# zehuichen123/Graph-DETR4D

Hardware: AMD Instinct MI355X
Metric: decoder_samples_per_sec_900q_T4 (higher is better)
Workload: dtype f32 (bf16x3 GEMMs)

## Files before the change

graph-detr4d_amd/_lib.py:

```python
import ctypes
import os
import threading

_HERE = os.path.dirname(os.path.abspath(__file__))
LIB_PATH = os.environ.get('GD4D_LIB_PATH') or os.path.join(_HERE, 'libgd4d.so')
ABI_VERSION = 56
PIXEL_MAJOR, HEAD_MAJOR = 0, 1

F32, BF16, F16 = 0, 1, 2

_c = ctypes
_vp, _i, _f = _c.c_void_p, _c.c_int, _c.c_float

SIGNATURES = {
    'gd4d_abi_version': (_i, []),
    'gd4d_error_string': (_c.c_char_p, [_i]),
    'gd4d_last_hip_error': (_c.c_char_p, []),
    'gd4d_trace_enable': (_i, [_vp]),
    'gd4d_cross_attn_fwd': (_i, [_vp, _vp, _vp, _vp, _vp, _vp, _vp, _vp, _f, _f, _vp, _vp, _vp,
                                 _i, _i, _i, _i, _i, _i, _i, _i, _i, _i, _vp, _vp]),
    'gd4d_pyramid_channels_last_fwd': (_i, [_vp, _vp, _vp, _i, _i, _i, _i, _i, _i, _vp]),
    'gd4d_cross_attn_agg_fwd': (_i, [_vp] * 8 + [_f, _f] + [_vp] * 4 + [_i] * 9 + [_vp] * 5),
    'gd4d_cross_attn_plan_bytes': (_c.c_size_t, [_i] * 5),
    'gd4d_cross_attn_plan_fwd': (_i, [_vp] * 6 + [_f, _f, _vp, _vp, _c.c_int64, _vp, _c.c_size_t, _vp, _vp, _vp] + [_i] * 7 + [_vp, _vp]),
# ... 40 lines not shown
    'gd4d_linear_fwd': (_i, [_vp] * 7 + [_i] * 9 + [_vp, _vp]),
    'gd4d_linear_group_fwd': (_i, [_vp] * 6 + [_i] * 4 + [_vp, _vp]),
    'gd4d_linear_ln_fwd': (_i, [_vp] * 9 + [_i] * 5 + [_f] + [_i] * 4 + [_vp]),
    'gd4d_small_linear_layernorm_fwd': (_i, [_vp] * 6 + [_i, _i, _i, _f, _i, _vp]),
    'gd4d_layernorm_fwd': (_i, [_vp] * 5 + [_i, _i, _f, _i, _vp]),
    'gd4d_mha_core_fwd': (_i, [_vp] * 5 + [_i] * 10 + [_f, _vp, _f, _vp, _vp]),
    'gd4d_mha_core_bwd': (_i, [_vp] * 11 + [_i] * 14 + [_f, _f, _vp, _vp]),
    'gd4d_mha_core_bwd_fill': (_i, [_vp] * 11 + [_i] * 14 + [_f, _f, _vp] + [_vp, _i, _vp, _vp] + [_i] * 4 + [_vp]),
    'gd4d_layernorm_bwd_workspace_bytes': (_c.c_size_t, [_i, _i]),
    'gd4d_layernorm_bwd': (_i, [_vp] * 9 + [_c.c_size_t, _i, _i, _f, _i, _vp]),
    'gd4d_inverse_sigmoid_fwd': (_i, [_vp, _vp, _c.c_int64, _vp]),
    'gd4d_inverse_sigmoid_bwd': (_i, [_vp, _vp, _vp, _vp, ctypes.c_int64, _vp]),
    'gd4d_layernorm_bwd_reduce_group': (_i, [_vp] * 4 + [_i, _i, _vp]),
    'gd4d_refine_reference_fwd': (_i, [_vp, _vp, _vp, _i, _i, _vp]),
    'gd4d_frustum_pe_input_fwd': (_i, [_vp, _vp, _vp, _i, _i, _i, _i, _f, _f, _f, _vp, _i, _i, _vp]),
    'gd4d_se_fuse_chlast_fwd': (_i, [_vp] * 5 + [_i] * 7 + [_vp]),
    'gd4d_sine_pe3d_fwd': (_i, [_vp, _vp, _vp, _vp, _vp, _i, _i, _i, _i, _i, _vp]),
    'gd4d_se_fuse_fwd': (_i, [_vp, _vp, _vp, _vp, _vp, _c.c_size_t, _vp]),
    'gd4d_split_bf16_fwd': (_i, [_vp, _vp, _vp, _c.c_size_t, _vp]),
    'gd4d_gemm_bf16x3_fwd': (_i, [_vp] * 5 + [_i] * 6 + [_vp]),
    'gd4d_image_job_bytes': (ctypes.c_size_t, []),
    'gd4d_chain_weight_image_group': (_i, [_vp, _i, _i, _vp]),
    'gd4d_gemm_tn_bf16x3_workspace_bytes': (ctypes.c_size_t, [ctypes.c_longlong, _i, _i]),
    'gd4d_gemm_tn_bf16x3': (_i, [_vp] * 5 + [ctypes.c_longlong] + [_i] * 5 + [_vp]),
    'gd4d_se_fuse_chlast_bwd': (_i, [_vp] * 6 + [_i] * 5 + [_vp]),
    'gd4d_knn_farthest_fwd': (_i, [_vp, _vp, _i, _i, _i, _i, _vp]),
    'gd4d_edge_conv_max_fwd': (_i, [_vp] * 6 + [_i] * 5 + [_vp]),
    'gd4d_box_head_fwd': (_i, [_vp, _vp, _vp, _f, _vp, _i, _i, _vp]),
    'gd4d_nms_free_decode_fwd': (_i, [_vp, _vp, _vp, _f, _vp, _vp, _vp, _vp, _i, _i, _i, _i, _i, _vp]),
    'gd4d_value_proj_multi_fwd': (_i, [_vp, _vp, _vp, _vp, _vp, _i, _i, _i, _i, _i, _i, _i, _i, _i, _vp, _c.c_size_t, _i, _vp]),
    'gd4d_chain_op_bytes': (_c.c_size_t, []),
    'gd4d_row_chain_fwd': (_i, [_vp, _i, _i, _vp]),
    'gd4d_row_chain2_fwd': (_i, [_vp, _i, _vp, _i, _i, _vp]),
    'gd4d_mha_core_presplit_fwd': (_i, [_vp] * 4 + [_i] * 5 + [_c.c_longlong, _c.c_longlong, _vp, _i, _f, _vp, _f, _vp, _vp]),
    'gd4d_xcd_placement_probe': (_i, [_vp, _i, _vp]),
    'gd4d_mlp2_image_bytes': (_c.c_size_t, [_i] * 3),
    'gd4d_mlp2_image': (_i, [_vp, _vp, _vp, _i, _i, _i, _vp, _vp]),
    'gd4d_mlp2_bf16x3_fwd': (_i, [_vp] * 4 + [_i] * 6 + [_vp]),
    'gd4d_mlp2_se_fuse_fwd': (_i, [_vp, _vp, _i, _i, _vp, _vp, _vp, _vp, _vp, _i, _i, _vp]),
    'gd4d_mlp2_frustum_fwd': (_i, [_vp, _vp, _i, _i, _c.c_float, _c.c_float, _i, _c.c_float, _vp, _vp, _vp, _vp, _i, _i, _vp]),
    'gd4d_mlp2_pe_se_fwd': (_i, [_vp, _vp, _vp, _i, _i, _c.c_float, _c.c_float, _i, _c.c_float, _vp, _vp, _vp, _i, _vp, _vp, _i, _vp, _vp,
                                  _vp, _vp]),
    'gd4d_adamw_flat_workspace_bytes': (_c.c_size_t, []),
    'gd4d_adamw_flat': (_i, [_vp] * 6 + [_c.c_size_t, _c.c_int64] + [_f] * 6 + [_vp]),
    'gd4d_adamw_recipe_flat_workspace_bytes': (_c.c_size_t, []),
    'gd4d_adamw_recipe_flat_state_bytes': (_c.c_size_t, []),
    'gd4d_adamw_recipe_flat': (_i, [_vp] * 5 + [_c.c_size_t, _vp, _c.c_size_t, _c.c_int64, _vp, _vp, _vp, _i, _vp]),
    'gd4d_chain_weight_image_bytes': (_c.c_size_t, [_i, _i]),
    'gd4d_chain_weight_image': (_i, [_vp, _i, _i, _vp, _vp]),
    'gd4d_chain_weight_image_exact_bytes': (_c.c_size_t, [_i, _i]),
    'gd4d_chain_weight_image_exact': (_i, [_vp, _i, _i, _vp, _vp]),
    'gd4d_linear_sum_assignment_batch': (_i, [_vp] * 4 + [_i, _vp, _vp, _i]),
    'gd4d_hungarian_assign_workspace_bytes': (_c.c_size_t, [_i] * 4),
    'gd4d_hungarian_assign_fwd': (_i, [_vp] * 5 + [_c.c_size_t] + [_i] * 5 + [_vp]),
    'gd4d_hungarian_assign_branches_workspace_bytes': (_c.c_size_t, [_i] * 5),
    'gd4d_hungarian_assign_branches_fwd': (_i, [_vp] * 9 + [_c.c_size_t] + [_i] * 8 + [_vp]),
    'gd4d_match_cost_fwd': (_i, [_vp] * 6 + [_i] * 8 + [_f] * 3 + [_vp]),
    'gd4d_head_loss_fwd_bwd': (_i, [_vp] * 10 + [_i] * 7 + [_f] * 3 + [_vp]),
    'gd4d_linear_bwd_weight': (_i, [_vp] * 4 + [_i] * 6 + [_vp]),
    'gd4d_linear_bwd_weight_group': (_i, [_vp] * 5 + [_i, _i, _vp]),
    'gd4d_value_proj_bwd_input': (_i, [_vp, _vp, _vp, _vp, _i, _i, _i, _i, _vp]),
    'gd4d_value_proj_bwd_weight_workspace_bytes': (_c.c_size_t, []),
    'gd4d_value_proj_bwd_weight': (_i, [_vp] * 6 + [_c.c_size_t, _i, _i, _i, _vp]),
    'gd4d_depth_net_image_bytes': (_c.c_size_t, [_i]),
    'gd4d_depth_net_image': (_i, [_vp, _i, _vp, _vp]),
    'gd4d_cam_gate_fwd': (_i, [_vp, _vp, _i, _i, _f] + [_vp] * 8 + [_i, _vp, _vp]),
# ... 117 lines not shown
```

graph-detr4d_amd/csrc/gd4d_rowchain.hip:

```cpp
#include <stdlib.h>

#include "gd4d_common.h"
#include "gd4d_bf16x3.h"
#include "gd4d_pyramid_fill.h"
#include "gd4d_mha_dropout.h"
#include "gd4d_value_proj_body.h"

namespace gd4d {

GD4D_TRACE_UNIT(rowchain)

constexpr int RC_M = 16;
#ifndef RC_WAVES_N
#define RC_WAVES_N 8
#endif
#ifndef RC_TILES_N
#define RC_TILES_N 2
#endif
constexpr int RC_WAVES = RC_WAVES_N;
#ifndef RC_KPERM
#define RC_KPERM 1
#endif
#ifndef RC_LD_N
#define RC_LD_N 520
// ... 526 lines not shown
  for (int r = 0; r < RC_ROWS_PER_WAVE; ++r) {
    const int m = min(m0 + RC_ROWS_PER_WAVE * wave + r, M - 1);
#pragma unroll
    for (int cb = 0; cb < 2; ++cb) {
      const int n = min(256 * cb + 4 * lane, N - 4);
      va[r][cb] = ga ? *reinterpret_cast<const float4*>(ga + (size_t)m * lda + n) : make_float4(0.f, 0.f, 0.f, 0.f);
      vb[r][cb] = gb ? *reinterpret_cast<const float4*>(gb + (size_t)m * ldb + n) : make_float4(0.f, 0.f, 0.f, 0.f);
    }
  }
#pragma unroll
  for (int r = 0; r < RC_ROWS_PER_WAVE; ++r) {
    const int row = RC_ROWS_PER_WAVE * wave + r;
#pragma unroll
    for (int cb = 0; cb < 2; ++cb) {
      const int n = 256 * cb + 4 * lane;
      if (n >= N) continue;
      float4 v = va[r][cb];
      if (!IS_ADD && (op.flags & GD4D_CHAIN_INV_SIGMOID)) { v.x = inv_sigmoid(v.x); v.y = inv_sigmoid(v.y); v.z = inv_sigmoid(v.z); v.w = inv_sigmoid(v.w); }
      v.x += vb[r][cb].x; v.y += vb[r][cb].y; v.z += vb[r][cb].z; v.w += vb[r][cb].w;
      if (IS_ADD) {
        const float4 s0 = *reinterpret_cast<const float4*>(&bufs[op.src][row][n]);
        v.x += s0.x; v.y += s0.y; v.z += s0.z; v.w += s0.w;
        if (op.res >= 0) {
          const float4 s1 = *reinterpret_cast<const float4*>(&bufs[op.res][row][n]);
          v.x += s1.x; v.y += s1.y; v.z += s1.z; v.w += s1.w;
        }
      }
      *reinterpret_cast<float4*>(&bufs[op.dst][row][(IS_ADD ? 0 : op.dst_col) + n]) = v;
      if (TRAIN && op.gout && m0 + row < M) *reinterpret_cast<float4*>(op.gout + (size_t)(m0 + row) * op.ldg + n) = v;
    }
  }
}

struct ChainProgram {
  int nops, M, nops2, split;
  ChainOp ops[GD4D_CHAIN_MAX_OPS];
};

#if defined(__HIP_DEVICE_COMPILE__)
typedef const __attribute__((address_space(4))) ChainProgram* rc_prog_ptr_t;
#else
typedef const ChainProgram* rc_prog_ptr_t;
#endif

template <bool TRAIN>
__device__ __forceinline__ void row_chain_body(const rc_prog_ptr_t pp, const int bx) {
  const int M = pp->M, split = pp->split;
  const int blocks = (M + RC_M - 1) / RC_M;
  if (split > 0 && bx >= blocks && bx < split) return;
  const bool second = split > 0 && bx >= split;
  const int op_base = second ? pp->nops : 0;
  const int nops = second ? pp->nops2 : pp->nops;
  const int wg = second ? bx - split : bx;
  const int wg_lo = second ? split : 0, wg_hi = wg_lo + blocks;
  extern __shared__ __attribute__((aligned(16))) char rc_smem[];
  float (*bufs)[RC_M][RC_LD] = reinterpret_cast<float (*)[RC_M][RC_LD]>(rc_smem);
  const int tid = threadIdx.x, lane = tid & 63, wave = tid >> 6;
  const int m0 = wg * RC_M;
  trace_mark_if(g_trace_rowchain, (second ? 7ull : 1ull) | ((unsigned long long)nops << 8), wg == 0);
#if RC_PREFETCH
  typedef __attribute__((address_space(3))) void rc_lds_void_t;
  typedef const __attribute__((address_space(1))) void rc_glb_void_t;
  rc_lds_void_t* rc_dump = (rc_lds_void_t*)(rc_smem + sizeof(float) * RC_BUFS * RC_M * RC_LD + 256 * wave);
  auto touch1 = [&](const char* q) { __builtin_amdgcn_global_load_lds((rc_glb_void_t*)q, rc_dump, 4, 0, 0); };
  const unsigned xcd = (unsigned)bx & 7u;
  const unsigned first = (unsigned)wg_lo + ((xcd - (unsigned)wg_lo) & 7u);
  const unsigned mine = ((unsigned)bx - first) >> 3, share = ((unsigned)wg_hi - 1u - first) / 8u + 1u;
  auto touch = [&](const void* base, size_t bytes) {
    if (!base || bytes < 4) return;
    const char* b = reinterpret_cast<const char*>(base);
    const unsigned pieces = (unsigned)((bytes + 63) / 64) + 1u;
    for (unsigned c = tid; c < pieces; c += 64 * RC_WAVES) touch1(b + min((size_t)c * 64, bytes - 4));
  };
  auto touch_small = [&](int from) {
    const int rows = min(RC_M, M - m0);
    for (int oi = from; oi < op_base + nops; ++oi) {
      const ChainOp& o = pp->ops[oi];
      const size_t nb = (size_t)o.N * 4;
      switch (o.kind) {
        case GD4D_CHAIN_LOAD:
          for (int r = 0; r < rows; ++r) {
            touch(o.p0 + (size_t)(m0 + r) * o.ld0, nb);
            if (o.p1) touch(o.p1 + (size_t)(m0 + r) * o.ld1, nb);
          }
          break;
        case GD4D_CHAIN_ADD:
          if (o.p2) for (int r = 0; r < rows; ++r) touch(o.p2 + (size_t)(m0 + r) * o.ld2, nb);
          break;
        case GD4D_CHAIN_GEMM: touch(o.p1, nb); break;
        case GD4D_CHAIN_HEADGEMM: touch(o.p1, nb); touch(o.p3 + (size_t)m0 * o.ld0, (size_t)rows * o.ld0 * 4); break;
        case GD4D_CHAIN_LAYERNORM: touch(o.p0, nb); touch(o.p1, nb); break;
        case GD4D_CHAIN_SMALL_LINEAR: touch(o.p0, nb * o.K); touch(o.p1, nb); break;
        case GD4D_CHAIN_REFINE: touch(o.p0 + (size_t)m0 * 3, (size_t)rows * 12); break;
        default: break;
      }
    }
  };
  auto touch_images = [&]() {
    for (int oi = op_base; oi < op_base + nops; ++oi) {
      if (pp->ops[oi].kind == GD4D_CHAIN_HEADGEMM) {
        const int rows = min(RC_M, M - m0);
        const char* a = reinterpret_cast<const char*>(pp->ops[oi].p2 + (size_t)m0 * pp->ops[oi].ld0 * pp->ops[oi].K);
        const unsigned pieces = (unsigned)rows * (unsigned)pp->ops[oi].ld0 * (unsigned)pp->ops[oi].K / 16u;
        for (unsigned c = tid; c < pieces; c += 64 * RC_WAVES) touch1(a + (size_t)c * 64);
      }
      if (pp->ops[oi].kind != GD4D_CHAIN_GEMM && pp->ops[oi].kind != GD4D_CHAIN_HEADGEMM) continue;
      const char* img = reinterpret_cast<const char*>(pp->ops[oi].p0);
      const unsigned chunks = (unsigned)((pp->ops[oi].N + 15) / 16) * (unsigned)(pp->ops[oi].K / 32) *
                              ((pp->ops[oi].flags & GD4D_CHAIN_EXACT) ? 48u : 32u);
      const unsigned lo = (unsigned)((unsigned long long)chunks * mine / share), hi = (unsigned)((unsigned long long)chunks * (mine + 1) / share);
      for (unsigned c = lo + tid; c < hi; c += 64 * RC_WAVES) touch1(img + (size_t)c * 64);
    }
  };
  int lead = 0;
  if (RC_PREFETCH & 4)
    while (lead < nops && pp->ops[op_base + lead].kind == GD4D_CHAIN_LOAD) ++lead;
  if (RC_PREFETCH & 2) touch_small(op_base + lead);
  if ((RC_PREFETCH & 1) && lead == 0) touch_images();
#endif
  __shared__ int rc_poison;
  if (tid == 0) rc_poison = 0;
  bool poisoned = false;
  for (int oi = op_base; oi < op_base + nops; ++oi) {
#if RC_PREFETCH
    if ((RC_PREFETCH & 1) && lead > 0 && oi == op_base + lead) touch_images();
#endif
    const ChainOp op = pp->ops[oi];
    switch (op.kind) {
      case GD4D_CHAIN_LOAD: {
        if ((op.N & 3) == 0 && (op.dst_col & 3) == 0) { rc_rows<false, TRAIN>(op, bufs, m0, M, lane, wave); break; }
        for (int e = tid; e < RC_M * op.N; e += 64 * RC_WAVES) {
          const int row = e / op.N, n = e - row * op.N;
          const int m = min(m0 + row, M - 1);
          float v = rc_act_in(op.p0[(size_t)m * op.ld0 + n], op.flags);
          if (op.p1) v += op.p1[(size_t)m * op.ld1 + n];
          bufs[op.dst][row][op.dst_col + n] = v;
          if (TRAIN && op.gout && m0 + row < M) op.gout[(size_t)(m0 + row) * op.ldg + n] = v;
        }
        break;
      }
      case GD4D_CHAIN_GEMM:
        if (op.flags & GD4D_CHAIN_EXACT) rc_gemm<true, TRAIN>(op, bufs, m0, M, lane, wave);
        else rc_gemm<false, TRAIN>(op, bufs, m0, M, lane, wave);
        break;
      case GD4D_CHAIN_HEADGEMM: rc_headgemm(op, bufs, m0, M, lane, wave); break;
      case GD4D_CHAIN_LAYERNORM: rc_layernorm(op, bufs, m0, M, lane, wave); break;
      case GD4D_CHAIN_ADD: rc_rows<true, TRAIN>(op, bufs, m0, M, lane, wave); break;
      case GD4D_CHAIN_DROPMASK: {
        if (!TRAIN) break;
        const uint32_t lo = reinterpret_cast<const uint32_t*>(op.p0)[0], hi = reinterpret_cast<const uint32_t*>(op.p0)[1];
// ... 275 lines not shown
      case GD4D_CHAIN_LN_BWD:
        if (!op.p0 || op.src < 0 || op.N <= 0 || op.N > RC_W) return GD4D_EINVAL;
        if (!op.p3 && (op.res < 0 || op.res == op.src || op.res == op.dst)) return GD4D_EINVAL;
        if (op.p3 && (!aligned16(op.p3) || (op.ld1 & 3) || op.ld1 < op.N)) return GD4D_EALIGN;
        if (op.dst < 0 && !op.gout && !op.p2) return GD4D_EINVAL;
        if ((op.flags & GD4D_CHAIN_RELU) && !op.p1) return GD4D_EINVAL;
        if (op.N % 64 != 0) return GD4D_EUNSUPPORTED;
        if (!aligned16(op.p0) || (op.p1 && !aligned16(op.p1)) || (op.gout && (!aligned16(op.gout) || (op.ldg & 3)))) return GD4D_EALIGN;
        break;
      case GD4D_CHAIN_ADD:
        if (op.src < 0 || op.dst < 0 || op.N <= 0 || op.N > RC_W || (op.N & 3)) return GD4D_EINVAL;
        if (op.p2 && (!aligned16(op.p2) || (op.ld2 & 3))) return GD4D_EALIGN;
        if (op.gout && (!aligned16(op.gout) || (op.ldg & 3))) return GD4D_EALIGN;
        break;
      case GD4D_CHAIN_SMALL_LINEAR:
        if (!op.p0 || op.src < 0 || op.dst < 0 || op.dst == op.src || op.K <= 0 || op.K > 8 || op.N <= 0 || op.N > RC_W)
          return GD4D_EINVAL;
        break;
      case GD4D_CHAIN_REFINE:
        if (op.src < 0 || !op.p0 || !op.gout || (op.dst >= 0 && op.dst == op.src)) return GD4D_EINVAL;
        break;
      case GD4D_CHAIN_SIGNAL:
        if (!op.gout || !two_programs || which != 1) return GD4D_EINVAL;
        break;
      case GD4D_CHAIN_WAIT:
        if (!op.p0 || !op.gout || !two_programs || which != 2 || i + 1 >= nops || program[i + 1].kind != GD4D_CHAIN_LOAD) return GD4D_EINVAL;
        break;
      default: return GD4D_EINVAL;
    }
  }
  return GD4D_OK;
}

static int rc_launch(const gd4d_chain_op* a, int na, const gd4d_chain_op* b, int nb, int M, void* stream,
                     const gd4d_chain_guest* guest = nullptr, const gd4d::FillGuest* fills = nullptr, int fill_workgroups = 0) {
  using namespace gd4d;
  if (!a || na <= 0 || M <= 0 || nb < 0 || (nb > 0 && !b)) return GD4D_EINVAL;
  if (na + nb > GD4D_CHAIN_MAX_OPS) return GD4D_EUNSUPPORTED;
  if (int rc = rc_validate(a, na, nb > 0 ? 1 : 0)) return rc;
  if (nb > 0)
    if (int rc = rc_validate(b, nb, 2)) return rc;
  for (int w = 0; w < 2; ++w)
    for (int i = 0; i < (w ? nb : na); ++i) {
      const gd4d_chain_op& op = (w ? b : a)[i];
      if (op.kind == GD4D_CHAIN_GEMM && (op.flags & GD4D_CHAIN_SPLIT_KV)) {
        const long long blocks = (M + RC_M - 1) / RC_M, heads = RC_COLS * RC_WAVES / 32;
        if (op.ld2 < heads * blocks * 512 || op.ld1 < heads * ((blocks + 1) / 2) * 1024) return GD4D_EINVAL;
      }
    }
  bool train = false;
  for (int w = 0; w < 2; ++w) {
    const gd4d_chain_op* pr = w ? b : a;
    for (int i = 0; i < (w ? nb : na); ++i) {
      const gd4d_chain_op& op = pr[i];
      train = train || op.kind == GD4D_CHAIN_LN_BWD || op.kind == GD4D_CHAIN_DROPMASK ||
              (op.kind == GD4D_CHAIN_GEMM && (op.flags & (GD4D_CHAIN_MASK_P2 | GD4D_CHAIN_DROPOUT))) ||
              ((op.kind == GD4D_CHAIN_LOAD || op.kind == GD4D_CHAIN_ADD || op.kind == GD4D_CHAIN_SMALL_LINEAR) && op.gout);
    }
  }
  VpaParams g{};
  if (guest) {
    if (train) return GD4D_EUNSUPPORTED;
    if (int rc = va_guest_params(guest, g)) return rc;
  }
  const size_t lds = sizeof(float) * RC_BUFS * RC_M * RC_LD + 256 * RC_WAVES + (train ? sizeof(float) * 8 * RC_W : 0);
  const void* kern = train ? reinterpret_cast<const void*>(row_chain_kernel<true>) : reinterpret_cast<const void*>(row_chain_kernel<false>);
  if (!allow_dynamic_lds(kern, (int)lds)) return GD4D_ELAUNCH;
  const int blocks = (M + RC_M - 1) / RC_M;
  ChainProgram prog{};
  const int split = nb > 0 ? (blocks + 7) & ~7 : 0;
  prog.nops = na; prog.M = M; prog.nops2 = nb; prog.split = split;
  for (int i = 0; i < na; ++i) prog.ops[i] = a[i];
  for (int i = 0; i < nb; ++i) prog.ops[na + i] = b[i];
  if (guest) {
    const int base = g.total;
    if (va_lds_bytes(1, false, RC_WAVES) > lds) return GD4D_EUNSUPPORTED;
    const int chain_wgs = nb > 0 ? split + blocks : blocks;
    const int gbase = chain_wgs;
    int cus = 256, dev = 0;
    if (hipGetDevice(&dev) != hipSuccess || hipDeviceGetAttribute(&cus, hipDeviceAttributeMultiprocessorCount, dev) != hipSuccess || cus <= 0) cus = 256;
    const int need = (base + RC_WAVES - 1) / RC_WAVES;
    int gcount = guest->workgroups > 0 ? guest->workgroups : cus;
    if (gcount < 8) gcount = 8;
    if (gcount > need) gcount = need;
    auto go = [&](auto kern) -> int {
      if (!allow_dynamic_lds(reinterpret_cast<const void*>(kern), (int)lds)) return GD4D_ELAUNCH;
      hipLaunchKernelGGL(kern, dim3(gbase + gcount), dim3(64 * RC_WAVES), lds, static_cast<hipStream_t>(stream), prog, g, gbase, gcount);
      return check_launch();
    };
    return g.in_chlast ? go(row_chain_guest_kernel<true>) : go(row_chain_guest_kernel<false>);
  }
  if (fills) {
    if (guest) return GD4D_EINVAL;
    const void* fk = reinterpret_cast<const void*>(row_chain_fill_kernel);
    const size_t flds = sizeof(float) * RC_BUFS * RC_M * RC_LD + 256 * RC_WAVES + sizeof(float) * 8 * RC_W;
    if (!allow_dynamic_lds(fk, (int)flds)) return GD4D_ELAUNCH;
    const int gbase = nb > 0 ? split + blocks : blocks;
    int cus = 256, dev = 0;
    if (hipGetDevice(&dev) != hipSuccess || hipDeviceGetAttribute(&cus, hipDeviceAttributeMultiprocessorCount, dev) != hipSuccess || cus <= 0) cus = 256;
    const int rows = fills->BQ[0] * fills->HH + (fills->hdr[1] ? fills->BQ[1] * fills->HH : 0);
    const int need = (rows + RC_WAVES - 1) / RC_WAVES;
    int gcount = fill_workgroups > 0 ? fill_workgroups : 2 * cus;
    if (gcount > need) gcount = need;
    if (gcount < 1) gcount = 1;
    hipLaunchKernelGGL(row_chain_fill_kernel, dim3(gbase + gcount), dim3(64 * RC_WAVES), flds, static_cast<hipStream_t>(stream), prog, *fills,
                       gbase, gcount);
    return check_launch();
  }
  if (train)
    hipLaunchKernelGGL(row_chain_kernel<true>, dim3(nb > 0 ? split + blocks : blocks), dim3(64 * RC_WAVES), lds, static_cast<hipStream_t>(stream), prog);
  else
    hipLaunchKernelGGL(row_chain_kernel<false>, dim3(nb > 0 ? split + blocks : blocks), dim3(64 * RC_WAVES), lds, static_cast<hipStream_t>(stream), prog);
  return check_launch();
}

extern "C" int gd4d_xcd_placement_probe(int32_t* out, int blocks, void* stream) {
  if (!out || blocks <= 0) return GD4D_EINVAL;
  hipLaunchKernelGGL(gd4d::xcd_placement_probe_kernel, dim3(blocks), dim3(64), 0, static_cast<hipStream_t>(stream), out);
  return gd4d::check_launch();
}

extern "C" int gd4d_row_chain_fwd(const gd4d_chain_op* program, int nops, int M, void* stream) {
  return rc_launch(program, nops, nullptr, 0, M, stream);
}

extern "C" int gd4d_row_chain2_fwd(const gd4d_chain_op* program_a, int nops_a, const gd4d_chain_op* program_b, int nops_b, int M,
                                   void* stream) {
  if (!program_b || nops_b <= 0) return GD4D_EINVAL;
  return rc_launch(program_a, nops_a, program_b, nops_b, M, stream);
}

extern "C" size_t gd4d_chain_guest_bytes(void) { return sizeof(gd4d_chain_guest); }

extern "C" int gd4d_row_chain_guest_fwd(const gd4d_chain_op* program_a, int nops_a, const gd4d_chain_op* program_b, int nops_b, int M,
                                        const gd4d_chain_guest* guest, void* stream) {
  if (!guest || nops_b < 0 || (nops_b > 0 && !program_b)) return GD4D_EINVAL;
  return rc_launch(program_a, nops_a, nops_b > 0 ? program_b : nullptr, nops_b, M, stream, guest);
}

extern "C" int gd4d_row_chain_fill_fwd(const gd4d_chain_op* program_a, int nops_a, const gd4d_chain_op* program_b, int nops_b, int M,
                                       const gd4d_fill_job* jobs, int njobs, const int32_t* start, void* records, int fill_B, int fill_N,
                                       int fill_Hh, int fill_P, int workgroups, void* stream) {
  using namespace gd4d;
  if (!jobs || njobs < 1 || njobs > 2 || !start || !records || fill_B <= 0 || fill_N <= 0 || fill_Hh <= 0) return GD4D_EINVAL;
  if (nops_b < 0 || (nops_b > 0 && !program_b) || workgroups < 0) return GD4D_EINVAL;
  if ((fill_P != kPoints && fill_P != 8) || fill_N > 64 || fill_B > 16 || fill_Hh > kPlanHdr) return GD4D_EUNSUPPORTED;
// ... 19 lines not shown
```

graph-detr4d_amd/ops.py:

```python
import ctypes
import functools
import inspect
import os
import weakref

import torch

from . import _lib


def _dev(t, name, dtype=None):
    if not t.is_cuda:
        raise _lib.Gd4dError(f'{name} must live on the GPU (no CPU fallback in graph-detr4d_amd)')
    if dtype is not None and t.dtype != dtype:
        raise TypeError(f'{name} must be {dtype}, got {t.dtype}')
    if not t.is_contiguous():
        raise ValueError(f'{name} must be contiguous')
    return ctypes.c_void_p(t.data_ptr())


def _stream():
    return ctypes.c_void_p(torch.cuda.current_stream().cuda_stream)


# ... 2180 lines not shown
    arr = (FillJob * len(jobs))(*[FillJob(_dev(pl.buf, 'plan', torch.uint8).value, _dev(sl, 'slots').value,
                                           None if pl.order is None else _order_ptr(pl.order, fb * pl.q).value, int(base), int(pl.q))
                                   for pl, sl, base in jobs])
    code = lib.gd4d_row_chain_fill_fwd(a, na, b, nb, int(m), arr, len(jobs), _dev(start, 'start', torch.int32), _dev(records, 'records'),
                                       fb, fn, fhh, int(jobs[0][0].points), 0, _stream())
    _lib.check(code, 'gd4d_row_chain_fill_fwd')


def row_chain_fwd(program, m, guest=None, fills=None):
    lib = _lib.load()
    arr = (ChainOp * len(program))(*program)
    if fills is not None:
        return _chain_fills(lib, arr, len(program), None, 0, m, fills)
    if guest is not None:
        code = lib.gd4d_row_chain_guest_fwd(arr, len(program), None, 0, int(m), ctypes.byref(guest), _stream())
        _lib.check(code, 'gd4d_row_chain_guest_fwd')
        return
    code = lib.gd4d_row_chain_fwd(arr, len(program), int(m), _stream())
    _lib.check(code, 'gd4d_row_chain_fwd')


def row_chain2_fwd(program_a, program_b, m, guest=None, fills=None):
    lib = _lib.load()
    a = (ChainOp * len(program_a))(*program_a)
    b = (ChainOp * len(program_b))(*program_b)
    if fills is not None:
        return _chain_fills(lib, a, len(program_a), b, len(program_b), m, fills)
    if guest is not None:
        code = lib.gd4d_row_chain_guest_fwd(a, len(program_a), b, len(program_b), int(m), ctypes.byref(guest), _stream())
        _lib.check(code, 'gd4d_row_chain_guest_fwd')
        return
    code = lib.gd4d_row_chain2_fwd(a, len(program_a), b, len(program_b), int(m), _stream())
    _lib.check(code, 'gd4d_row_chain2_fwd')


def mha_core_presplit_fwd(q, kv, num_heads, attn_mask=None, want_lse=False, dropout_p=0., seed=None):
    lib = _lib.load()
    lq, b, c = q.shape
    _, _, _, _, _, _, kind, mptr, keep = _mha_args(q, q, q, num_heads, attn_mask)
    if b != 1 or lq != kv.m or c != kv.c or num_heads != kv.heads:
        raise ValueError('mha_core_presplit_fwd: batch 1, the planes of these rows')
    if not q.is_cuda or q.dtype != torch.float32 or q.stride(2) != 1:
        raise _lib.Gd4dError('q must be a float32 GPU tensor with unit channel stride')
    d = c // num_heads
    out = torch.empty(lq, 1, c, device=q.device, dtype=torch.float32)
    lse = torch.empty(lq, 1, num_heads, device=q.device, dtype=torch.float32) if want_lse else None
    sptr = _mha_seed(dropout_p, seed, q.device)
    code = lib.gd4d_mha_core_presplit_fwd(ctypes.c_void_p(q.data_ptr()), ctypes.c_void_p(kv.k.data_ptr()),
                                          ctypes.c_void_p(kv.v.data_ptr()), _dev(out, 'out'), lq, num_heads, d, q.stride(0), c,
                                          kv.k[0].numel(), kv.v[0].numel(), mptr, kind, 1.0 / (d ** 0.5),
                                          None if lse is None else _dev(lse, 'lse'), float(dropout_p), sptr, _stream())
    _lib.check(code, 'gd4d_mha_core_presplit_fwd')
    return (out, lse) if want_lse else out


class RequestRef(ctypes.Structure):
    _fields_ = [('binding', ctypes.c_int32), ('reserved', ctypes.c_int32), ('value', ctypes.c_int64)]


class RequestPatch(ctypes.Structure):
    _fields_ = [('table', ctypes.c_int32), ('binding', ctypes.c_int32), ('offset', ctypes.c_int64), ('add', ctypes.c_int64)]


class RequestBinding(ctypes.Union):
    _fields_ = [('ptr', ctypes.c_void_p), ('scalar', ctypes.c_double)]

# ... 1003 lines not shown
```

include/gd4d.h:

```cpp
#ifndef GD4D_H_
#define GD4D_H_

#include <stddef.h>
#include <stdint.h>

#ifdef __cplusplus
extern "C" {
#endif

#define GD4D_ABI_VERSION 56

enum { GD4D_F32 = 0, GD4D_BF16 = 1, GD4D_F16 = 2 };

enum { GD4D_LAYOUT_PIXEL_MAJOR = 0, GD4D_LAYOUT_HEAD_MAJOR = 1 };

enum { GD4D_VP_PRECISION_F32 = 0, GD4D_VP_PRECISION_BF16 = 1 };

enum {
  GD4D_OK = 0,
  GD4D_EINVAL = -1,
  GD4D_EUNSUPPORTED = -2,
  GD4D_EALIGN = -3,
  GD4D_ELAUNCH = -4,
  GD4D_EWORKSPACE = -5
// ... 178 lines not shown
#define GD4D_CHAIN_MASK_P2 64
#define GD4D_CHAIN_DROPOUT 128
#define GD4D_CHAIN_SPLIT_KV 256
#define GD4D_CHAIN_SPLIT_KV_KEEP 512
#define GD4D_CHAIN_ADD_GOUT 1024
#define GD4D_CHAIN_MAX_OPS 32
typedef struct gd4d_chain_op {
  int32_t kind, src, dst, res;
  int32_t K, N, flags, dst_col;
  int32_t ld0, ld1, ld2, ldg;
  float eps;
  int32_t reserved;
  const float* p0;
  const float* p1;
  const float* p2;
  float* gout;
  const float* p3;
} gd4d_chain_op;
size_t gd4d_chain_op_bytes(void);
size_t gd4d_chain_weight_image_bytes(int N, int K);
int gd4d_chain_weight_image(const float* weight, int N, int K, void* image, void* stream);
size_t gd4d_chain_weight_image_exact_bytes(int N, int K);
int gd4d_chain_weight_image_exact(const float* weight, int N, int K, void* image, void* stream);
#define GD4D_IMAGE_JOBS_MAX 1024
typedef struct gd4d_image_job {
  const float* seg[3];
  int32_t rows[3];
  int32_t cols, transposed, planes, frag0, reserved;
  void* image;
} gd4d_image_job;
size_t gd4d_image_job_bytes(void);
int gd4d_chain_weight_image_group(const gd4d_image_job* jobs_device, int count, int total_frags, void* stream);
int gd4d_row_chain_fwd(const gd4d_chain_op* program, int nops, int M, void* stream);
int gd4d_row_chain2_fwd(const gd4d_chain_op* program_a, int nops_a, const gd4d_chain_op* program_b, int nops_b, int M,
                        void* stream);

typedef struct gd4d_chain_guest {
  const void* feats[GD4D_MAX_LEVELS];
  int32_t level_hw[2 * GD4D_MAX_LEVELS];
  int32_t L, R, chlast, workgroups;
  const void* image;
  void* out;
} gd4d_chain_guest;
size_t gd4d_chain_guest_bytes(void);
size_t gd4d_value_proj_image_bytes(void);
int gd4d_value_proj_image(const float* weight, const float* bias, void* image, void* stream);
int gd4d_row_chain_guest_fwd(const gd4d_chain_op* program_a, int nops_a, const gd4d_chain_op* program_b, int nops_b, int M,
                             const gd4d_chain_guest* guest, void* stream);
int gd4d_value_proj_guest_fwd(const gd4d_chain_guest* job, int max_cus, void* stream);

int gd4d_mha_core_presplit_fwd(const float* q, const void* k_planes, const void* v_planes, float* out, int L, int H, int D,
                               int ldq, int ldo, long long k_plane_stride, long long v_plane_stride, const void* mask,
                               int mask_kind, float scale, float* lse, float drop_p, const void* seed, void* stream);

size_t gd4d_mlp2_image_bytes(int K1, int H, int N2);
int gd4d_mlp2_image(const float* w1, const float* b1, const float* w2, int K1, int H, int N2, void* image, void* stream);
int gd4d_mlp2_bf16x3_fwd(const float* x, const void* image, const float* b2, float* out, int M, int K1, int H, int N2, int ldx,
                         int ldo, void* stream);
int gd4d_mlp2_se_fuse_fwd(const void* const* feats, const int32_t* level_hw, int L, int R, const void* image, const float* b2,
                          const float* pe, const float* sine, void* const* outs, int C, int H, void* stream);
int gd4d_mlp2_frustum_fwd(const float* img2lidar, const int32_t* level_hw, int L, int R, float pad_h, float pad_w, int D,
                          float depth_start, const double* pc_range, const void* image, const float* b2, float* out, int H, int ldo,
                          void* stream);
int gd4d_mlp2_pe_se_fwd(const float* img2lidar, const void* const* feats, const int32_t* level_hw, int L, int R, float pad_h,
                        float pad_w, int D, float depth_start, const double* pc_range, const void* pe_image, const float* pe_b2,
                        int pe_H, const void* se_image, const float* se_b2, int se_H, const float* sine, void* const* outs,
// ... 309 lines not shown
```

Measured before the change: 678.8.

## Precompute cold-read prefetch list on host and warm kernel-argument program

Replaces the per-op in-kernel prefetch walk with a host-computed list of read-only segments that no chain op writes. Each block touches those segments with one load per thread by row and column. A scalar-load burst also pre-reads the program's op records out of the kernel argument segment. By default only that scalar warming runs (GD4D_CHAIN_WARM defaults to 1), so the cold-segment prefetch is disabled unless the environment variable enables it. The program structure grows, and its size is asserted to fit the 4 KB argument segment.

```diff
diff --git a/graph-detr4d_amd/_lib.py b/graph-detr4d_amd/_lib.py
--- a/graph-detr4d_amd/_lib.py
+++ b/graph-detr4d_amd/_lib.py
@@ -96,6 +96,7 @@
     'gd4d_chain_op_bytes': (_c.c_size_t, []),
     'gd4d_row_chain_fwd': (_i, [_vp, _i, _i, _vp]),
     'gd4d_row_chain2_fwd': (_i, [_vp, _i, _vp, _i, _i, _vp]),
+    'gd4d_row_chain_cold_list': (_i, [_vp, _i, _vp, _i, _i, _i, _vp, _i]),
     'gd4d_mha_core_presplit_fwd': (_i, [_vp] * 4 + [_i] * 5 + [_c.c_longlong, _c.c_longlong, _vp, _i, _f, _vp, _f, _vp, _vp]),
     'gd4d_xcd_placement_probe': (_i, [_vp, _i, _vp]),
     'gd4d_mlp2_image_bytes': (_c.c_size_t, [_i] * 3),
diff --git a/graph-detr4d_amd/csrc/gd4d_rowchain.hip b/graph-detr4d_amd/csrc/gd4d_rowchain.hip
--- a/graph-detr4d_amd/csrc/gd4d_rowchain.hip
+++ b/graph-detr4d_amd/csrc/gd4d_rowchain.hip
@@ -582,10 +582,21 @@
   }
 }
 
+struct ColdSeg {
+  const char* base;
+  int32_t row_stride;
+  uint32_t packed;
+};
+constexpr int RC_COLD = 16;
+
 struct ChainProgram {
   int nops, M, nops2, split;
+  int warm, ncold[2], pad;
   ChainOp ops[GD4D_CHAIN_MAX_OPS];
+  ColdSeg cold[2][RC_COLD];
 };
+static_assert(sizeof(ChainProgram) <= 4096, "the program travels in the 4 KB kernel argument segment");
+static_assert(sizeof(ChainProgram) + sizeof(VpaParams) + 8 <= 4096 && sizeof(ChainProgram) + sizeof(FillGuest) + 8 <= 4096, "... with the guests' parameters behind it");
 
 #if defined(__HIP_DEVICE_COMPILE__)
 typedef const __attribute__((address_space(4))) ChainProgram* rc_prog_ptr_t;
@@ -608,6 +619,21 @@
   const int tid = threadIdx.x, lane = tid & 63, wave = tid >> 6;
   const int m0 = wg * RC_M;
   trace_mark_if(g_trace_rowchain, (second ? 7ull : 1ull) | ((unsigned long long)nops << 8), wg == 0);
+  const int warm = pp->warm;
+#if defined(__HIP_DEVICE_COMPILE__)
+  if (warm & 1) {
+    typedef const __attribute__((address_space(4))) char* rc_k_ptr_t;
+    const rc_k_ptr_t k0 = (rc_k_ptr_t)pp;
+    unsigned sink = 0;
+    auto burst = [&](unsigned lo, unsigned hi) {
+      for (unsigned o = lo & ~63u; o < hi; o += 64u) asm volatile("s_load_dword %0, %1, 0x0" : "+s"(sink) : "s"(k0 + o) : "memory");
+    };
+    burst((unsigned)(offsetof(ChainProgram, ops) + sizeof(ChainOp) * op_base), (unsigned)(offsetof(ChainProgram, ops) + sizeof(ChainOp) * (op_base + nops)));
+    burst((unsigned)(offsetof(ChainProgram, cold) + sizeof(ColdSeg) * RC_COLD * (second ? 1 : 0)),
+          (unsigned)(offsetof(ChainProgram, cold) + sizeof(ColdSeg) * (RC_COLD * (second ? 1 : 0) + pp->ncold[second ? 1 : 0])));
+    asm volatile("s_waitcnt lgkmcnt(0)" : "+s"(sink) : : "memory");
+  }
+#endif
 #if RC_PREFETCH
   typedef __attribute__((address_space(3))) void rc_lds_void_t;
   typedef const __attribute__((address_space(1))) void rc_glb_void_t;
@@ -616,34 +642,17 @@
   const unsigned xcd = (unsigned)bx & 7u;
   const unsigned first = (unsigned)wg_lo + ((xcd - (unsigned)wg_lo) & 7u);
   const unsigned mine = ((unsigned)bx - first) >> 3, share = ((unsigned)wg_hi - 1u - first) / 8u + 1u;
-  auto touch = [&](const void* base, size_t bytes) {
-    if (!base || bytes < 4) return;
-    const char* b = reinterpret_cast<const char*>(base);
-    const unsigned pieces = (unsigned)((bytes + 63) / 64) + 1u;
-    for (unsigned c = tid; c < pieces; c += 64 * RC_WAVES) touch1(b + min((size_t)c * 64, bytes - 4));
-  };
-  auto touch_small = [&](int from) {
-    const int rows = min(RC_M, M - m0);
-    for (int oi = from; oi < op_base + nops; ++oi) {
-      const ChainOp& o = pp->ops[oi];
-      const size_t nb = (size_t)o.N * 4;
-      switch (o.kind) {
-        case GD4D_CHAIN_LOAD:
-          for (int r = 0; r < rows; ++r) {
-            touch(o.p0 + (size_t)(m0 + r) * o.ld0, nb);
-            if (o.p1) touch(o.p1 + (size_t)(m0 + r) * o.ld1, nb);
-          }
-          break;
-        case GD4D_CHAIN_ADD:
-          if (o.p2) for (int r = 0; r < rows; ++r) touch(o.p2 + (size_t)(m0 + r) * o.ld2, nb);
-          break;
-        case GD4D_CHAIN_GEMM: touch(o.p1, nb); break;
-        case GD4D_CHAIN_HEADGEMM: touch(o.p1, nb); touch(o.p3 + (size_t)m0 * o.ld0, (size_t)rows * o.ld0 * 4); break;
-        case GD4D_CHAIN_LAYERNORM: touch(o.p0, nb); touch(o.p1, nb); break;
-        case GD4D_CHAIN_SMALL_LINEAR: touch(o.p0, nb * o.K); touch(o.p1, nb); break;
-        case GD4D_CHAIN_REFINE: touch(o.p0 + (size_t)m0 * 3, (size_t)rows * 12); break;
-        default: break;
-      }
+  auto touch_cold = [&]() {
+    const int which = second ? 1 : 0, n = pp->ncold[which];
+    for (int e = 0; e < n; ++e) {
+      const char* base = pp->cold[which][e].base;
+      const int stride = pp->cold[which][e].row_stride;
+      const unsigned pk = pp->cold[which][e].packed;
+      const unsigned bytes = pk & 0xfffffu, rows = (pk >> 20) & 31u, sh = (pk >> 25) & 15u;
+      const unsigned pieces = (bytes + 63u) / 64u + ((pk >> 29) & 1u ? 0u : 1u);
+      const unsigned r = (unsigned)tid >> sh, c = (unsigned)tid & ((1u << sh) - 1u);
+      if (r < rows && m0 + (int)r < M && c < pieces)
+        touch1(base + (size_t)(m0 + (int)r) * (size_t)stride + min(c * 64u, bytes - 4u));
     }
   };
   auto touch_images = [&]() {
@@ -665,7 +674,7 @@
   int lead = 0;
   if (RC_PREFETCH & 4)
     while (lead < nops && pp->ops[op_base + lead].kind == GD4D_CHAIN_LOAD) ++lead;
-  if (RC_PREFETCH & 2) touch_small(op_base + lead);
+  if (warm & 2) touch_cold();
   if ((RC_PREFETCH & 1) && lead == 0) touch_images();
 #endif
   __shared__ int rc_poison;
@@ -1007,22 +1016,101 @@
   return GD4D_OK;
 }
 
+namespace {
+struct RcSeg { const char* base; long long stride, bytes; int rows; };
+struct RcRange { const char* lo; const char* hi; };
+
+int rc_cold_list(const gd4d_chain_op* a, int na, const gd4d_chain_op* b, int nb, int M, int which, RcSeg* out, int cap) {
+  using namespace gd4d;
+  const long long blocks = (M + RC_M - 1) / RC_M;
+  RcRange wr[3 * GD4D_CHAIN_MAX_OPS];
+  int nw = 0;
+  auto wrote = [&](const void* p, long long bytes) {
+    if (p && bytes > 0) wr[nw++] = RcRange{static_cast<const char*>(p), static_cast<const char*>(p) + bytes};
+  };
+  auto wrote_rows = [&](const void* p, long long ld, long long n) { wrote(p, ((long long)(M - 1) * ld + n) * 4); };
+  for (int w = 0; w < 2; ++w)
+    for (int i = 0; i < (w ? nb : na); ++i) {
+      const gd4d_chain_op& op = (w ? b : a)[i];
+      switch (op.kind) {
+        case GD4D_CHAIN_GEMM:
+          if (op.flags & GD4D_CHAIN_SPLIT_OUT) {
+            wrote_rows(op.gout, op.ldg, op.ldg); wrote_rows(op.p2, op.ld2, op.ld2); wrote_rows(op.p3, op.ld1, op.ld1);
+          } else {
+            wrote_rows(op.gout, op.ldg, op.N);
+            if (op.flags & GD4D_CHAIN_SPLIT_KV) { wrote(op.p2, 4ll * op.ld2); wrote(op.p3, 4ll * op.ld1); }
+          }
+          break;
+        case GD4D_CHAIN_HEADGEMM: if (!(op.flags & GD4D_CHAIN_ADD_GOUT)) wrote_rows(op.gout, op.ldg, op.N); break;
+        case GD4D_CHAIN_REFINE: wrote(op.gout, 12ll * M); break;
+        case GD4D_CHAIN_LN_BWD: wrote_rows(op.gout, op.ldg, op.N); wrote(op.p2, blocks * 2 * op.N * 4); break;
+        case GD4D_CHAIN_SIGNAL: wrote(op.gout, blocks * 4); break;
+        case GD4D_CHAIN_WAIT: wrote(op.gout, 4); wrote(op.p0, blocks * 4); break;
+        default: wrote_rows(op.gout, op.ldg, op.N); break;
+      }
+    }
+  int n = 0;
+  auto add = [&](const void* p, long long stride, long long bytes, int rows) {
+    const char* base = static_cast<const char*>(p);
+    if (!base || bytes < 4 || (bytes & 3) || bytes >= (1ll << 20) || ((uintptr_t)base & 3) || (stride & 3) || stride < 0 || stride > 0x7fffffffll) return;
+    const char* hi = base + (rows > 1 ? (long long)(M - 1) * stride : 0) + bytes;
+    for (int i = 0; i < nw; ++i)
+      if (base < wr[i].hi && wr[i].lo < hi) return;
+    for (int i = 0; i < n; ++i)
+      if (out[i].base == base && out[i].stride == stride && out[i].bytes == bytes && out[i].rows == rows) return;
+    if (n < cap) out[n++] = RcSeg{base, stride, bytes, rows};
+  };
+  auto param = [&](const void* p, long long bytes) { add(p, 0, bytes, 1); };
+  auto rows = [&](const void* p, long long ld, long long cols) { add(p, ld * 4, cols * 4, RC_M); };
+  const gd4d_chain_op* pr = which ? b : a;
+  bool waited = false;
+  for (int i = 0; i < (which ? nb : na); ++i) {
+    const gd4d_chain_op& op = pr[i];
+    switch (op.kind) {
+      case GD4D_CHAIN_WAIT: waited = true; break;
+      case GD4D_CHAIN_LOAD:
+        if (waited) break;
+        rows(op.p0, op.ld0, op.N); rows(op.p1, op.ld1, op.N);
+        break;
+      case GD4D_CHAIN_ADD: rows(op.p2, op.ld2, op.N); break;
+      case GD4D_CHAIN_GEMM:
+        param(op.p1, 4ll * op.N);
+        if (op.flags & GD4D_CHAIN_DROPOUT) param(op.p3, 8);
+        if (op.flags & (GD4D_CHAIN_SPLIT_OUT | GD4D_CHAIN_SPLIT_KV)) break;
+        rows(op.p2, op.ld2, op.N);
+        if (!(op.flags & GD4D_CHAIN_DROPOUT)) rows(op.p3, op.ld1, op.N);
+        break;
+      case GD4D_CHAIN_HEADGEMM:
+        param(op.p1, 4ll * op.N);
+        rows(op.p3, op.ld0, op.ld0);
+        if (op.flags & GD4D_CHAIN_ADD_GOUT) rows(op.gout, op.ldg, op.N);
+        break;
+      case GD4D_CHAIN_LAYERNORM:
+        param(op.p0, 4ll * op.N); param(op.p1, 4ll * op.N);
+        if (op.res >= 0) rows(op.p2, op.ld2, op.N);
+        break;
+      case GD4D_CHAIN_SMALL_LINEAR: param(op.p0, 4ll * op.N * op.K); param(op.p1, 4ll * op.N); break;
+      case GD4D_CHAIN_REFINE: rows(op.p0, 3, 3); break;
+      case GD4D_CHAIN_LN_BWD: param(op.p0, 4ll * op.N); param(op.p1, 4ll * op.N); rows(op.p3, op.ld1, op.N); break;
+      case GD4D_CHAIN_DROPMASK: param(op.p0, 8); break;
+      default: break;
+    }
+  }
+  return n;
+}
+
+int rc_warm_bits() {
+  const char* e = getenv("GD4D_CHAIN_WARM");
+  return (e && e[0] >= '0' && e[0] <= '3' && !e[1]) ? e[0] - '0' : 1;
+}
+}
+
+static int rc_check_args(const gd4d_chain_op* a, int na, const gd4d_chain_op* b, int nb, int M);
+
 static int rc_launch(const gd4d_chain_op* a, int na, const gd4d_chain_op* b, int nb, int M, void* stream,
                      const gd4d_chain_guest* guest = nullptr, const gd4d::FillGuest* fills = nullptr, int fill_workgroups = 0) {
   using namespace gd4d;
-  if (!a || na <= 0 || M <= 0 || nb < 0 || (nb > 0 && !b)) return GD4D_EINVAL;
-  if (na + nb > GD4D_CHAIN_MAX_OPS) return GD4D_EUNSUPPORTED;
-  if (int rc = rc_validate(a, na, nb > 0 ? 1 : 0)) return rc;
-  if (nb > 0)
-    if (int rc = rc_validate(b, nb, 2)) return rc;
-  for (int w = 0; w < 2; ++w)
-    for (int i = 0; i < (w ? nb : na); ++i) {
-      const gd4d_chain_op& op = (w ? b : a)[i];
-      if (op.kind == GD4D_CHAIN_GEMM && (op.flags & GD4D_CHAIN_SPLIT_KV)) {
-        const long long blocks = (M + RC_M - 1) / RC_M, heads = RC_COLS * RC_WAVES / 32;
-        if (op.ld2 < heads * blocks * 512 || op.ld1 < heads * ((blocks + 1) / 2) * 1024) return GD4D_EINVAL;
-      }
-    }
+  if (int rc = rc_check_args(a, na, b, nb, M)) return rc;
   bool train = false;
   for (int w = 0; w < 2; ++w) {
     const gd4d_chain_op* pr = w ? b : a;
@@ -1047,6 +1135,20 @@
   prog.nops = na; prog.M = M; prog.nops2 = nb; prog.split = split;
   for (int i = 0; i < na; ++i) prog.ops[i] = a[i];
   for (int i = 0; i < nb; ++i) prog.ops[na + i] = b[i];
+  prog.warm = rc_warm_bits();
+  for (int w = 0; w < (nb > 0 ? 2 : 1) && (prog.warm & 2); ++w) {
+    RcSeg seg[RC_COLD];
+    const int n = rc_cold_list(a, na, b, nb, M, w, seg, RC_COLD);
+    for (int i = 0; i < n; ++i) {
+      const unsigned bytes = (unsigned)seg[i].bytes;
+      const bool lines = ((uintptr_t)seg[i].base & 63) == 0 && (seg[i].stride & 63) == 0;
+      const unsigned pieces = (bytes + 63u) / 64u + (lines ? 0u : 1u);
+      unsigned sh = 0;
+      while ((1u << sh) < pieces) ++sh;
+      prog.cold[w][i] = ColdSeg{seg[i].base, (int32_t)seg[i].stride, bytes | (unsigned)seg[i].rows << 20 | sh << 25 | (lines ? 1u << 29 : 0u)};
+    }
+    prog.ncold[w] = n;
+  }
   if (guest) {
     const int base = g.total;
     if (va_lds_bytes(1, false, RC_WAVES) > lds) return GD4D_EUNSUPPORTED;
@@ -1087,6 +1189,42 @@
   else
     hipLaunchKernelGGL(row_chain_kernel<false>, dim3(nb > 0 ? split + blocks : blocks), dim3(64 * RC_WAVES), lds, static_cast<hipStream_t>(stream), prog);
   return check_launch();
+}
+
+static int rc_check_args(const gd4d_chain_op* a, int na, const gd4d_chain_op* b, int nb, int M) {
+  using namespace gd4d;
+  if (!a || na <= 0 || M <= 0 || nb < 0 || (nb > 0 && !b)) return GD4D_EINVAL;
+  if (na + nb > GD4D_CHAIN_MAX_OPS) return GD4D_EUNSUPPORTED;
+  if (int rc = rc_validate(a, na, nb > 0 ? 1 : 0)) return rc;
+  if (nb > 0)
+    if (int rc = rc_validate(b, nb, 2)) return rc;
+  for (int w = 0; w < 2; ++w)
+    for (int i = 0; i < (w ? nb : na); ++i) {
+      const gd4d_chain_op& op = (w ? b : a)[i];
+      if (op.kind == GD4D_CHAIN_GEMM && (op.flags & GD4D_CHAIN_SPLIT_KV)) {
+        const long long blocks = (M + RC_M - 1) / RC_M, heads = RC_COLS * RC_WAVES / 32;
+        if (op.ld2 < heads * blocks * 512 || op.ld1 < heads * ((blocks + 1) / 2) * 1024) return GD4D_EINVAL;
+      }
+    }
+  return GD4D_OK;
+}
+
+extern "C" int gd4d_row_chain_cold_list(const gd4d_chain_op* program_a, int nops_a, const gd4d_chain_op* program_b, int nops_b, int M,
+                                        int which, gd4d_chain_cold_seg* out, int capacity) {
+  using namespace gd4d;
+  if ((which != 0 && which != 1) || (which == 1 && nops_b <= 0) || !out || capacity <= 0) return GD4D_EINVAL;
+  if (int rc = rc_check_args(program_a, nops_a, nops_b > 0 ? program_b : nullptr, nops_b, M)) return rc;
+  RcSeg seg[RC_COLD];
+  const int n = rc_cold_list(program_a, nops_a, program_b, nops_b, M, which, seg, RC_COLD);
+  int k = 0;
+  for (; k < n && k < capacity; ++k) {
+    out[k].base = seg[k].base;
+    out[k].row_stride_bytes = (int32_t)seg[k].stride;
+    out[k].bytes_per_row = (int32_t)seg[k].bytes;
+    out[k].rows = seg[k].rows;
+    out[k].reserved = 0;
+  }
+  return k;
 }
 
 extern "C" int gd4d_xcd_placement_probe(int32_t* out, int blocks, void* stream) {
diff --git a/graph-detr4d_amd/ops.py b/graph-detr4d_amd/ops.py
--- a/graph-detr4d_amd/ops.py
+++ b/graph-detr4d_amd/ops.py
@@ -2236,6 +2236,39 @@
         return
     code = lib.gd4d_row_chain2_fwd(a, len(program_a), b, len(program_b), int(m), _stream())
     _lib.check(code, 'gd4d_row_chain2_fwd')
+
+
+class ChainColdSeg(ctypes.Structure):
+    _fields_ = [('base', ctypes.c_void_p), ('row_stride_bytes', ctypes.c_int32), ('bytes_per_row', ctypes.c_int32),
+                ('rows', ctypes.c_int32), ('reserved', ctypes.c_int32)]
+
+
+def row_chain_cold_list(program_a, m, program_b=None, which=0, capacity=16):
+    a = (ChainOp * len(program_a))(*program_a)
+    b = (ChainOp * len(program_b))(*program_b) if program_b else None
+    out = (ChainColdSeg * max(int(capacity), 1))()
+    n = _lib.load().gd4d_row_chain_cold_list(a, len(program_a), b, len(program_b) if program_b else 0, int(m), int(which), out, int(capacity))
+    if n < 0:
+        _lib.check(n, 'gd4d_row_chain_cold_list')
+    return [(int(out[i].base or 0), int(out[i].row_stride_bytes), int(out[i].bytes_per_row), int(out[i].rows)) for i in range(n)]
+
+
+class chain_warm:
+
+    def __init__(self, on):
+        self.on, self.prev = (3 if on else 0) if isinstance(on, bool) else int(on), None
+
+    def __enter__(self):
+        import os
+        self.prev = os.environ.get('GD4D_CHAIN_WARM')
+        os.environ['GD4D_CHAIN_WARM'] = str(self.on)
+
+    def __exit__(self, *exc):
+        import os
+        if self.prev is None:
+            os.environ.pop('GD4D_CHAIN_WARM', None)
+        else:
+            os.environ['GD4D_CHAIN_WARM'] = self.prev
 
 
 def mha_core_presplit_fwd(q, kv, num_heads, attn_mask=None, want_lse=False, dropout_p=0., seed=None):
diff --git a/include/gd4d.h b/include/gd4d.h
--- a/include/gd4d.h
+++ b/include/gd4d.h
@@ -234,6 +234,12 @@
 size_t gd4d_image_job_bytes(void);
 int gd4d_chain_weight_image_group(const gd4d_image_job* jobs_device, int count, int total_frags, void* stream);
 int gd4d_row_chain_fwd(const gd4d_chain_op* program, int nops, int M, void* stream);
+typedef struct gd4d_chain_cold_seg {
+  const void* base;
+  int32_t row_stride_bytes, bytes_per_row, rows, reserved;
+} gd4d_chain_cold_seg;
+int gd4d_row_chain_cold_list(const gd4d_chain_op* program_a, int nops_a, const gd4d_chain_op* program_b, int nops_b, int M, int which,
+                             gd4d_chain_cold_seg* out, int capacity);
 int gd4d_row_chain2_fwd(const gd4d_chain_op* program_a, int nops_a, const gd4d_chain_op* program_b, int nops_b, int M,
                         void* stream);
 
```

Result: no change. 679.3 (median of 4 runs) (+0.1%).
